# rayanirban/DiffSplitting

Hardware: AMD Instinct MI355X
Metric: sampled images/sec (2000-step 128x128 SR3) (higher is better)
Workload: dtype bf16; 1 GPU; sr_sr3_16_128: GaussianDiffusion.p_sample_loop, 16->128 SR3 UNet (97.8M params), T=2000 linear schedule; one step = UNet forward + posterior update of the batch; batch_per_gpu=16, global_batch=16, image=128x128x3, sample_steps=2000, parallelism=1 independent replicas, final RCCL all-gather, hipgraph=True, streams=1, noise=device Philox4x32-10, weights=random-init, seed 0

## Files before the change

### diffsplitting_amd/csrc/dsx_conv.hip

```cpp
#include "dsx_kernels.h"
#include <algorithm>
#include <cstdlib>
#include <mutex>
#include <type_traits>
#include <utility>

#ifndef DSX_WS_DEPTH_EXPR
#define DSX_WS_DEPTH_EXPR (bm == 64 ? 5 : (bm == 256 ? 2 : (ks == 1 ? 3 : 4)))
#endif
#ifndef DSX_PRE_RESID_EXPR
#define DSX_PRE_RESID_EXPR (NB == 1 && MB <= 2)
#endif
#ifndef DSX_PFF_EXPR
#define DSX_PFF_EXPR (NB == 2 ? 3 : 6)
#endif
#ifndef DSX_WS_K0_EXPR
#define DSX_WS_K0_EXPR 64
#endif
#ifndef DSX_EPI_PRIO_COND
#define DSX_EPI_PRIO_COND false
#endif
#ifndef DSX_STAMP_CVT_COND
#define DSX_STAMP_CVT_COND (tiC == 2 && gC == 0)
#endif
// ... 1075 lines not shown
  auto tile_pixel0 = [&](const TilePos& t) __attribute__((always_inline)) -> int {
    return (t.b * a.Ho + (t.ty << a.th_log2)) * a.Wo + (t.tx << a.tw_log2);
  };
  TilePos cur;
  {
    const int q1 = (int)fastdiv((unsigned)p0, a.mg_tiles_x);
    cur.b = (int)fastdiv((unsigned)p0, a.mg_per_img);
    cur.tx = p0 - q1 * a.tiles_x;
    cur.ty = q1 - cur.b * a.tiles_y;
  }
  TilePos nxt = cur;
  tile_advance(nxt);
  TilePos nn = nxt;
  tile_advance(nn);

  auto load_aff = [&](int b, int slot) __attribute__((always_inline)) {
    if (a.gn_scale == nullptr || tid * 4 >= C) return;
    float* dst = aff_base + (size_t)slot * (AFFB / 4);
    *(float4*)(dst + tid * 4) = *(const float4*)(a.gn_scale + (size_t)b * C + tid * 4);
    *(float4*)(dst + C + tid * 4) = *(const float4*)(a.gn_shift + (size_t)b * C + tid * 4);
  };
  TilePos n3 = nn;
  tile_advance(n3);
  load_aff(cur.b, 0);
  if (ntile > 1) load_aff(nxt.b, 1);
  if (ntile > 2) load_aff(nn.b, 2);

  constexpr int NR = 8 / CPU;
  const float4 zero4 = make_float4(0.f, 0.f, 0.f, 0.f);
  float4 addv[NB][2], affv[2];
  constexpr bool PRE_RESID = DSX_PRE_RESID_EXPR;
  uint4 residv[PRE_RESID ? MB : 1][NB][2][NR];
#pragma unroll
  for (int nb = 0; nb < NB; ++nb)
#pragma unroll
    for (int j = 0; j < 2; ++j) addv[nb][j] = zero4;
  if (a.bias && !a.film) {
#pragma unroll
    for (int nb = 0; nb < NB; ++nb)
#pragma unroll
      for (int j = 0; j < 2; ++j) addv[nb][j] = *(const float4*)(a.bias + nbase + 32 * nb + 4 * j);
  }
#pragma unroll
  for (int mb = 0; mb < (PRE_RESID ? MB : 1); ++mb)
#pragma unroll
    for (int nb = 0; nb < NB; ++nb)
#pragma unroll
      for (int ph = 0; ph < 2; ++ph)
#pragma unroll
        for (int q = 0; q < NR; ++q) residv[mb][nb][ph][q] = make_uint4(0u, 0u, 0u, 0u);
  affv[0] = affv[1] = zero4;
  auto prefetch_epilogue = [&](const TilePos& t, bool want_aff, int b_aff) __attribute__((always_inline)) {
    if (a.film) {
#pragma unroll
      for (int nb = 0; nb < NB; ++nb)
#pragma unroll
        for (int j = 0; j < 2; ++j)
          addv[nb][j] = *(const float4*)(a.film + (size_t)t.b * a.film_bs + nbase + 32 * nb + 4 * j);
    }
    if (PRE_RESID && a.resid) {
      const int r0 = tile_pixel0(t) * a.resid_ld;
#pragma unroll
      for (int mb = 0; mb < (PRE_RESID ? MB : 1); ++mb)
#pragma unroll
        for (int ph = 0; ph < 2; ++ph) {
          const DT* rp = (const DT*)a.resid + (r0 + rrow[mb] + ph * r16);
#pragma unroll
          for (int nb = 0; nb < NB; ++nb)
#pragma unroll
            for (int q = 0; q < NR; ++q) residv[mb][nb][ph][q] = *(const uint4*)(rp + 32 * nb + CPU * q);
        }
    }
    if (want_aff && a.gn_scale != nullptr && tid * 4 < C) {
      affv[0] = *(const float4*)(a.gn_scale + (size_t)b_aff * C + tid * 4);
      affv[1] = *(const float4*)(a.gn_shift + (size_t)b_aff * C + tid * 4);
    }
  };
  prefetch_epilogue(cur, ntile > 3, n3.b);

  constexpr bool PF_OK = !(NB == 2 && KS == 3);
  unsigned fin_pf_acc = 0u;
  if constexpr (PF_OK) fin_pf_acc = l2_prefetch_fold(l2_prefetch(a.pf, blockIdx.x, gridDim.x, tid, 256));
  if constexpr (KS == 1) {
    if (a.fin_on) {
      fin_pf_acc |= l2_prefetch_fold(l2_prefetch(a.fin.pf, blockIdx.x, gridDim.x, tid, 256));
      const int nitems = a.fin.B * a.fin.groups;
      for (int item = (int)blockIdx.x * 4 + wave; item < nitems; item += (int)gridDim.x * 4)
        gn_finalize_item<1>(a.fin, item % a.fin.B, item / a.fin.B, lane, nullptr);
    }
  }

  if constexpr (NBUF >= 3) {
    if (tid < 8) ((unsigned*)(lds + NBUF * BUFB + 3 * AFFB + NSLOT * RAWB))[tid] = 0u;
  }
  ws_barrier();
  if constexpr (NBUF == 2) ws_barrier();
  DSX_STAMP_T(0, tid == 0);
  int g = 0, ti = 0, aslot = 0;
  int ibuf = 0;
  constexpr int NPAIR = NSTEP / 2;
  constexpr int NF = 2 * MB;
  constexpr int FT = NPAIR * NF;
  constexpr int PFF = (DSX_PFF_EXPR) < FT ? (DSX_PFF_EXPR) : FT - 1;
  static_assert(PFF >= 1 && PFF < FT && PFF <= 15, "lgkmcnt is 4 bits");
  constexpr int RP = D > NSTEP ? D / NSTEP : 1;
  if constexpr (RP == 1) {
    for (int v = 0; v < total; ++v) {
      constexpr int R0 = 0;
#define DSX_WS_ITEM_NEXT continue
#include "dsx_conv_ws_item.inc"
#undef DSX_WS_ITEM_NEXT
    }
  } else {
    for (int v0 = 0; v0 < total; v0 += RP)
      static_for<RP>([&](auto rc_) __attribute__((always_inline)) {
        constexpr int R0 = decltype(rc_)::value * NSTEP;
        const int v = v0 + decltype(rc_)::value;
        if (v >= total) return;
#define DSX_WS_ITEM_NEXT return
#include "dsx_conv_ws_item.inc"
#undef DSX_WS_ITEM_NEXT
      });
  }
  if constexpr (PF_OK) l2_prefetch_retire(a.pf, fin_pf_acc);
}


template <typename DT, int KS, int NPH>
__global__ __launch_bounds__(512, 1) void k_conv_img(const ConvArgs a) {
  constexpr int KC = Chunk<DT>::KC;
  constexpr int CPU = Unit<DT>::N;
  constexpr int ES = (int)sizeof(DT);
  constexpr int TAPS = KS * KS, PAD = KS / 2, PW = 8 + 2 * PAD;
  constexpr int PIXB = 80;
  constexpr int RB = KS == 3 ? 896 : 640;
  constexpr int IMGB = PW * RB;
  constexpr int NSTEP = TAPS * 2;
  constexpr int D = NSTEP;
  constexpr int MAXP = NPH;
  constexpr bool ALLW = NPH == 2;
  static_assert(NSTEP % D == 0, "ring depth divides the steps of a phase");
  extern __shared__ __attribute__((aligned(16))) unsigned char lds[];

  const int tid = threadIdx.x, lane = tid & 63;
  const int wave = __builtin_amdgcn_readfirstlane(tid >> 6);
  const int li = lane & 31, lh = lane >> 5;
  const int nb = blockIdx.x % a.nblocks, b = blockIdx.x / a.nblocks;
  const int C = a.C0 + a.C1;
  const int nphase = NPH != 8 ? NPH : C / (8 * KC);
  unsigned char* img = lds + wave * (2 * IMGB);
  float* aff = (float*)(lds + 8 * 2 * IMGB) + wave * (8 * 2 * KC);

  DSX_STAMP(0);
  if (KS == 3) {
    for (int q = lane; q < 360; q += 64) {
      const int bufi = q >= 180, r = q - 180 * bufi, bp = r / 5, u = r - 5 * bp;
      int py, px2;
      if (bp < 10) { py = 0; px2 = bp; }
      else if (bp < 20) { py = 9; px2 = bp - 10; }
      else { py = 1 + ((bp - 20) >> 1); px2 = ((bp - 20) & 1) ? 9 : 0; }
      *(uint4*)(img + bufi * IMGB + py * RB + px2 * PIXB + u * 16) = make_uint4(0u, 0u, 0u, 0u);
    }
  }

  auto load_raw = [&](int p, uint4 (&raw)[4]) __attribute__((always_inline)) {
    const int c0 = (p * 8 + wave) * KC;
    const bool first = c0 < a.C0;
    const char* src = (const char*)(first ? a.src0 : a.src1);
    const int Cs = first ? a.C0 : a.C1, cl = first ? c0 : c0 - a.C0;
#pragma unroll
    for (int i = 0; i < 4; ++i) {
      const int q = lane + 64 * i, px = q >> 2, u = q & 3;
      raw[i] = *(const uint4*)(src + (((size_t)b * 64 + px) * Cs + cl + u * CPU) * ES);
    }
  };
  auto convert_store = [&](int p, const uint4 (&raw)[4]) __attribute__((always_inline)) {
    unsigned char* buf = img + (p & 1) * IMGB;
    const int u = lane & 3;
    float sc[CPU], sh[CPU];
    if (a.has_gn) {
#pragma unroll
      for (int j = 0; j < CPU; ++j) { sc[j] = aff[p * 2 * KC + u * CPU + j]; sh[j] = aff[p * 2 * KC + KC + u * CPU + j]; }
    }
#pragma unroll
    for (int i = 0; i < 4; ++i) {
      const int px = (lane + 64 * i) >> 2;
      float v[CPU];
      Unit<DT>::unpack(raw[i], v);
      if (a.has_gn) affine_vec(v, sc, sh);
      if (a.swish) swish_vec(v);
      *(uint4*)(buf + ((px >> 3) + PAD) * RB + ((px & 7) + PAD) * PIXB + u * 16) = Unit<DT>::pack(v);
    }
  };

  uint2 glo[MAXP], ghi[MAXP];
  float gg[MAXP], gb[MAXP];
  if (a.has_gn) {
#pragma unroll
    for (int p = 0; p < MAXP; ++p) {
      const int pp = p < nphase ? p : nphase - 1;
      const int c0 = (pp * 8 + wave) * KC, cb = c0 & ~63, c = cb + lane;
      const bool first = cb < a.C0;
      const char* part = (const char*)(first ? a.gn_part0 : a.gn_part1);
      const int nch = first ? a.gn_nchunk0 : a.gn_nchunk1, pf32 = first ? a.gn_pf32_0 : a.gn_pf32_1;
      const int Cs = first ? a.C0 : a.C1, cl = first ? c : c - a.C0;
      const char* e = part + (((size_t)b * nch) * Cs + cl) * (pf32 ? 8 : 16);
      glo[p] = *(const uint2*)e;
      ghi[p] = *(const uint2*)(e + 8);
      gg[p] = a.gn_gamma[c]; gb[p] = a.gn_beta[c];
    }
  }
  uint4 raw0[4], raw1[4];
  load_raw(0, raw0);
  if (nphase > 1) load_raw(1, raw1);

  const unsigned char* wbase = (const unsigned char*)a.wpack + (size_t)nb * a.kchunks * (NSTEP * 1024) + lane * 16;
  int pn = 0, sn = 0;
  auto load_w = [&]() __attribute__((always_inline)) -> uint4 {
    const uint4 v = *(const uint4*)(wbase + ((size_t)(pn * 8 + wave) * NSTEP + sn) * 1024);
    if (++sn == NSTEP) { sn = 0; ++pn; }
    return v;
  };
  uint4 wq[D], wq1[ALLW ? D : 1];
#pragma unroll
  for (int j = 0; j < D; ++j) wq[j] = load_w();
  if constexpr (ALLW) {
    if (nphase > 1) {
#pragma unroll
      for (int j = 0; j < D; ++j) wq1[j] = load_w();
    }
  }
  DSX_STAMP(1);

  if (a.has_gn) {
    const int cpg = C / a.gn_groups;
    double gs[MAXP], gq[MAXP];
#pragma unroll
    for (int p = 0; p < MAXP; ++p) {
      const int pp = p < nphase ? p : nphase - 1;
      const int cb = ((pp * 8 + wave) * KC) & ~63, c = cb + lane;
      const bool first = cb < a.C0;
      const int nch = first ? a.gn_nchunk0 : a.gn_nchunk1, pf32 = first ? a.gn_pf32_0 : a.gn_pf32_1;
      const double d0 = __builtin_bit_cast(double, ((unsigned long long)glo[p].y << 32) | glo[p].x);
      const double d1 = __builtin_bit_cast(double, ((unsigned long long)ghi[p].y << 32) | ghi[p].x);
      gs[p] = pf32 ? (double)__builtin_bit_cast(float, glo[p].x) : d0;
      gq[p] = pf32 ? (double)__builtin_bit_cast(float, glo[p].y) : d1;
      if (nch > 1 && p < nphase) {
        const char* part = (const char*)(first ? a.gn_part0 : a.gn_part1);
        const int Cs = first ? a.C0 : a.C1, cl = first ? c : c - a.C0;
        for (int k = 1; k < nch; ++k) {
          const size_t idx = (((size_t)b * nch + k) * Cs + cl) * 2;
          if (pf32) { const float2 v = *(const float2*)((const float*)part + idx); gs[p] += v.x; gq[p] += v.y; }
          else { const double2 v = *(const double2*)((const double*)part + idx); gs[p] += v.x; gq[p] += v.y; }
        }
      }
      const StatPivot& piv = first ? a.gn_piv0 : a.gn_piv1;
      if (piv.bias || piv.film)
        stat_unshift(gs[p], gq[p], (double)stat_pivot(piv, b, first ? c : c - a.C0), (double)(a.Hs * a.Ws));
    }
    const float inv_n = 1.0f / (64.0f * (float)cpg);
#pragma unroll
    for (int p = 0; p < MAXP; ++p) {
      if (p < nphase) {
        const int c0 = (p * 8 + wave) * KC, c = (c0 & ~63) + lane;
        float s = (float)gs[p], q = (float)gq[p];
        for (int o = 1; o < cpg; o <<= 1) { s += __shfl_xor(s, o, 64); q += __shfl_xor(q, o, 64); }
        const double mean = (double)s * (double)inv_n;
        double var = (double)q * (double)inv_n - mean * mean;
        if (var < 0) var = 0;
        const float rstd = __builtin_amdgcn_rsqf((float)var + a.gn_eps);
        const float meanf = (float)mean;
        if (c >= c0 && c < c0 + KC) {
          const float sc = rstd * gg[p];
          aff[p * 2 * KC + (c - c0)] = sc;
          aff[p * 2 * KC + KC + (c - c0)] = gb[p] - meanf * sc;
        }
      }
    }
  }
  const PfAcc pf_acc = l2_prefetch(a.pf, blockIdx.x, gridDim.x, tid, 512);
  DSX_STAMP(2);
  __builtin_amdgcn_s_waitcnt(0xC07F);
  convert_store(0, raw0);
  if (nphase > 1) convert_store(1, raw1);
  DSX_STAMP(3);

  int abase[2][KS];
#pragma unroll
  for (int mb = 0; mb < 2; ++mb) {
    const int m = mb * 32 + li;
#pragma unroll
    for (int dy = 0; dy < KS; ++dy) abase[mb][dy] = ((m >> 3) + dy) * RB + (m & 7) * PIXB + lh * 16;
  }
  f32x16 acc[2];
#pragma unroll
  for (int mb = 0; mb < 2; ++mb)
#pragma unroll
    for (int r = 0; r < 16; ++r) acc[mb][r] = 0.f;

  for (int p = 0; p < nphase; ++p) {
    const unsigned char* buf = img + (p & 1) * IMGB;
    if (p + 2 < nphase) load_raw(p + 2, raw0);
    const bool more = p + 1 < nphase;
    static_for<NSTEP>([&](auto sc_) __attribute__((always_inline)) {
      constexpr int s = decltype(sc_)::value;
      constexpr int tap = s >> 1, fs = s & 1, dy = tap / KS, dx = tap % KS;
      uint4 wcur = wq[s % D];
      if constexpr (ALLW) {
        if (p == 1) wcur = wq1[s % D];
      } else {
        if (more) wq[s % D] = load_w();
      }
#pragma unroll
      for (int mb = 0; mb < 2; ++mb) {
        const f32x4_t px = *(const f32x4_t*)(buf + abase[mb][dy] + dx * PIXB + fs * 32);
        acc[mb] = mfma_step<DT>(wcur, px, acc[mb]);
      }
    });
    if (p + 2 < nphase) convert_store(p + 2, raw0);
    DSX_STAMP(4 + p);
  }

  const int px = tid >> 3, cg = (tid & 7) * 4;
  const int n0 = nb * 32 + cg;
  const size_t opix = (size_t)b * 64 + px;
  float4 eb = make_float4(0.f, 0.f, 0.f, 0.f), ef = eb;
  float er[4] = {0.f, 0.f, 0.f, 0.f};
  if (a.bias) eb = *(const float4*)(a.bias + n0);
  if (a.film) ef = *(const float4*)(a.film + (size_t)b * a.film_bs + n0);
  if (a.resid) {
#pragma unroll
    for (int j = 0; j < 4; ++j) er[j] = act_load<DT>(a.resid, opix * a.resid_ld + n0 + j);
  }
  __syncthreads();
  DSX_STAMP(12);
  float* part = (float*)lds;
#pragma unroll
  for (int mb = 0; mb < 2; ++mb)
#pragma unroll
    for (int j = 0; j < 4; ++j)
      *(float4*)(part + ((wave * 2 + mb) * 64 + lane) * 20 + 4 * j) =
          make_float4(acc[mb][4 * j], acc[mb][4 * j + 1], acc[mb][4 * j + 2], acc[mb][4 * j + 3]);
  __syncthreads();
  DSX_STAMP(13);
  const int mbo = px >> 5, lo = (px & 31) + 32 * (cg >> 4), r0 = cg & 15;
  float x[4] = {0.f, 0.f, 0.f, 0.f};
#pragma unroll
  for (int w = 0; w < 8; ++w) {
    const float4 t = *(const float4*)(part + ((w * 2 + mbo) * 64 + lo) * 20 + r0);
    x[0] += t.x; x[1] += t.y; x[2] += t.z; x[3] += t.w;
  }
  x[0] += eb.x; x[1] += eb.y; x[2] += eb.z; x[3] += eb.w;
  x[0] += ef.x; x[1] += ef.y; x[2] += ef.z; x[3] += ef.w;
#pragma unroll
  for (int j = 0; j < 4; ++j) x[j] += er[j];
  const int okind = a.out_bf16;
  if (okind == 0) {
    *(float4*)((float*)a.out + opix * a.out_ld + n0) = make_float4(x[0], x[1], x[2], x[3]);
  } else {
    uint2 w2;
    if (okind == 1) { w2.x = pack_bf16x2(x[0], x[1]); w2.y = pack_bf16x2(x[2], x[3]); }
    else { w2.x = pack_f16x2(x[0], x[1]); w2.y = pack_f16x2(x[2], x[3]); }
    *(uint2*)((unsigned short*)a.out + opix * a.out_ld + n0) = w2;
  }
  DSX_STAMP(14);
  if (a.stat_part != nullptr) {
    float s1[4], s2[4];
#pragma unroll
    for (int j = 0; j < 4; ++j) { s1[j] = x[j]; s2[j] = x[j] * x[j]; }
#pragma unroll
    for (int o = 8; o < 64; o <<= 1)
#pragma unroll
      for (int j = 0; j < 4; ++j) { s1[j] += __shfl_xor(s1[j], o, 64); s2[j] += __shfl_xor(s2[j], o, 64); }
    __syncthreads();
    float* red = (float*)lds;
    if (lane < 8) {
#pragma unroll
      for (int j = 0; j < 4; ++j) { red[(wave * 32 + cg + j) * 2] = s1[j]; red[(wave * 32 + cg + j) * 2 + 1] = s2[j]; }
    }
    __syncthreads();
    if (tid < 64) {
      const int ch = tid >> 1, k = tid & 1;
      float t = 0.f;
#pragma unroll
      for (int w = 0; w < 8; ++w) t += red[(w * 32 + ch) * 2 + k];
      a.stat_part[((size_t)b * a.Cout + nb * 32 + ch) * 2 + k] = t;
    }
  }
  l2_prefetch_retire(a.pf, pf_acc);
  DSX_STAMP(15);
}

static size_t conv_img_lds(int dtype, int ks) {
  const int KC = dtype != 0 ? 32 : 16;
  const int pw = ks == 3 ? 10 : 8, rb = ks == 3 ? 896 : 640;
  return (size_t)8 * 2 * pw * rb + (size_t)8 * 8 * 2 * KC * sizeof(float);
}
bool conv_img_applicable(int dtype, int ks, int stride, const ConvArgs& a, bool gn, int gn_groups) {
  if (stride != 1 || a.up || !(ks == 1 || ks == 3)) return false;
  if (a.Hs != 8 || a.Ws != 8 || a.Ho != 8 || a.Wo != 8) return false;
  const int KC = dtype != 0 ? 32 : 16, C = a.C0 + a.C1;
  if (a.C0 % (8 * KC) || a.C1 % (8 * KC) || C / (8 * KC) > 8 || C < 8 * KC) return false;
  if (a.Cout % 32 || (a.out_ld & 3) || (a.resid && (a.resid_ld & 3))) return false;
  if (gn) {
    if (gn_groups < 1 || C % gn_groups) return false;
    const int cpg = C / gn_groups;
    if (cpg > 64 || (cpg & (cpg - 1)) || a.C0 % cpg) return false;
  }
  return true;
}


template <typename DT>
__global__ __launch_bounds__(256) void k_conv_first(const ConvArgs a) {
  constexpr bool F32 = sizeof(DT) == 4;
  constexpr int ES = (int)sizeof(DT);
  constexpr int KSTEP = F32 ? 2 : 16;
  constexpr int NS16 = 4;
  __shared__ __attribute__((aligned(16))) unsigned char sm[18 * 18 * 7 * 4 + 64 * 4];
  DT* patch = (DT*)sm;
  int* kofft = (int*)(sm + 18 * 18 * 7 * 4);

  const int tid = threadIdx.x, lane = tid & 63;
  const int wave = __builtin_amdgcn_readfirstlane(tid >> 6);
  const int li = lane & 31, lh = lane >> 5;
  const int Cin = a.C0 + a.C1, K = 9 * Cin;
  const int tiles_x = a.Wo >> 4, tiles_y = a.Ho >> 4;
  const int t = blockIdx.x % (tiles_x * tiles_y), b = blockIdx.x / (tiles_x * tiles_y);
  const int ty = t / tiles_x, tx = t - ty * tiles_x;
  const int oy0 = ty * 16, ox0 = tx * 16;
  const int NBLK = (a.Cout + 31) >> 5;

  for (int e = tid; e < 18 * 18 * Cin; e += 256) {
    const int c = e % Cin, pp = e / Cin, px = pp % 18, py = pp / 18;
    const int iy = oy0 + py - 1, ix = ox0 + px - 1;
    DT v = (DT)0.f;
    if (iy >= 0 && iy < a.Hs && ix >= 0 && ix < a.Ws) {
      const size_t pix = ((size_t)b * a.Hs + iy) * a.Ws + ix;
      v = c < a.C0 ? ((const DT*)a.src0)[pix * a.C0 + c] : ((const DT*)a.src1)[pix * a.C1 + (c - a.C0)];
    }
    patch[e] = v;
  }
  if (F32 && tid < 64) {
    const int k = tid < K ? tid : 0;
    const int tap = k / Cin, c = k - tap * Cin;
    kofft[tid] = ((tap / 3) * 18 + (tap % 3)) * Cin + c;
  }
  int koff[F32 ? 1 : NS16 * 8];
  if constexpr (!F32) {
#pragma unroll
    for (int s = 0; s < NS16; ++s)
#pragma unroll
      for (int j = 0; j < 8; ++j) {
        int k = 16 * s + 8 * lh + j;
        if (k >= K) k = 0;
        const int tap = k / Cin, c = k - tap * Cin;
        koff[s * 8 + j] = (((tap / 3) * 18 + (tap % 3)) * Cin + c) * 2;
      }
  }
  uint4 wf[F32 ? 1 : 2 * NS16];
  if constexpr (!F32) {
#pragma unroll
    for (int nb = 0; nb < 2; ++nb)
#pragma unroll
      for (int s = 0; s < NS16; ++s)
        wf[nb * NS16 + s] = nb < NBLK ? ((const uint4*)a.wpack)[(nb * NS16 + s) * 64 + lane] : make_uint4(0u, 0u, 0u, 0u);
  }
  __syncthreads();

  f32x16 acc[2][2];
#pragma unroll
  for (int mb = 0; mb < 2; ++mb)
#pragma unroll
    for (int nb = 0; nb < 2; ++nb)
#pragma unroll
      for (int r = 0; r < 16; ++r) acc[mb][nb][r] = 0.f;

#pragma unroll
  for (int mb = 0; mb < 2; ++mb) {
    const int m = (wave * 2 + mb) * 32 + li;
    const int base = ((m >> 4) * 18 + (m & 15)) * Cin;
    if constexpr (F32) {
      const int nsteps = (K + 1) >> 1;
      const float* wp = (const float*)a.wpack;
      for (int s = 0; s < nsteps; ++s) {
        const float pv = ((const float*)patch)[base + kofft[2 * s + lh]];
#pragma unroll
        for (int nb = 0; nb < 2; ++nb) {
          if (nb < NBLK) acc[mb][nb] = __builtin_amdgcn_mfma_f32_32x32x2f32(wp[(nb * 32 + s) * 64 + lane], pv, acc[mb][nb], 0, 0, 0);
        }
      }
    } else {
      const unsigned char* pb = (const unsigned char*)patch + base * 2;
#pragma unroll
      for (int s = 0; s < NS16; ++s) {
        unsigned w4[4];
#pragma unroll
        for (int q = 0; q < 4; ++q) {
          const unsigned lo = *(const unsigned short*)(pb + koff[s * 8 + 2 * q]);
          const unsigned hi = *(const unsigned short*)(pb + koff[s * 8 + 2 * q + 1]);
          w4[q] = lo | (hi << 16);
        }
        const f32x4_t px = __builtin_bit_cast(f32x4_t, make_uint4(w4[0], w4[1], w4[2], w4[3]));
#pragma unroll
        for (int nb = 0; nb < 2; ++nb)
          if (nb < NBLK) acc[mb][nb] = mfma_step<DT>(wf[nb * NS16 + s], px, acc[mb][nb]);
      }
    }
  }
  (void)KSTEP; (void)ES;

  const int okind = a.out_bf16;
#pragma unroll
  for (int nb = 0; nb < 2; ++nb) {
    const int nbase = nb * 32 + 16 * lh;
    if (nb >= NBLK) continue;
    float s1[16], s2[16];
#pragma unroll
    for (int r = 0; r < 16; ++r) { s1[r] = 0.f; s2[r] = 0.f; }
    const bool live = nbase < a.Cout;
#pragma unroll
    for (int mb = 0; mb < 2; ++mb) {
      const int m = (wave * 2 + mb) * 32 + li;
      const size_t opix = ((size_t)b * a.Ho + (oy0 + (m >> 4))) * a.Wo + (ox0 + (m & 15));
      float x[16], pv[16];
#pragma unroll
      for (int r = 0; r < 16; ++r) { x[r] = acc[mb][nb][r]; pv[r] = 0.f; }
      if (live) {
        if (a.bias) {
#pragma unroll
          for (int j = 0; j < 4; ++j) { const float4 tt = *(const float4*)(a.bias + nbase + 4 * j); pv[4 * j] = tt.x; pv[4 * j + 1] = tt.y; pv[4 * j + 2] = tt.z; pv[4 * j + 3] = tt.w; }
#pragma unroll
          for (int r = 0; r < 16; ++r) x[r] += pv[r];
        }
        store16<true>(a.out, opix * a.out_ld + nbase, x, okind, 16);
#pragma unroll
        for (int r = 0; r < 16; ++r) { const float d = x[r] - pv[r]; s1[r] += d; s2[r] += d * d; }
      }
    }
    if (a.stat_part != nullptr) {
      float w1 = row16_fold(s1, lane), w2 = row16_fold(s2, lane);
      w1 += __shfl_xor(w1, 16, 64);
      w2 += __shfl_xor(w2, 16, 64);
      const int nch = tiles_x * tiles_y * 4, chunk = t * 4 + wave;
      const int n = nbase + row16_fold_reg(li);
      if (li < 16 && n < a.Cout) {
        float* pp = a.stat_part + (((size_t)b * nch + chunk) * a.Cout + n) * 2;
        pp[0] = w1; pp[1] = w2;
      }
    }
  }
}

bool conv_first_applicable(int ks, int stride, const ConvArgs& a, bool gn) {
  const int C = a.C0 + a.C1;
  return ks == 3 && stride == 1 && !a.up && !gn && !a.swish && C >= 1 && C <= 7 && a.Cout >= 16 && a.Cout <= 64 &&
         (a.Cout & 15) == 0 && (a.Ho & 15) == 0 && (a.Wo & 15) == 0 && a.Ho == a.Hs && a.Wo == a.Ws && a.out_ld == a.Cout;
}
hipError_t launch_conv_first(int dtype, const ConvArgs& a, hipStream_t st) {
  const unsigned grid = (unsigned)(a.B * (a.Ho >> 4) * (a.Wo >> 4));
  if (dtype == 1) hipLaunchKernelGGL(k_conv_first<__bf16>, dim3(grid), dim3(256), 0, st, a);
  else if (dtype == 2) hipLaunchKernelGGL(k_conv_first<_Float16>, dim3(grid), dim3(256), 0, st, a);
  else hipLaunchKernelGGL(k_conv_first<float>, dim3(grid), dim3(256), 0, st, a);
  return hipGetLastError();
}

enum ConvFamily { FAM_MFMA, FAM_WS, FAM_IMG };
struct ConvVariant {
  int family, dtype, tile, ks, stride, cpg;
  void (*kern)(const ConvArgs);
  int block, lds_cap;
  int MB, WM, WN, NB;
  int max_px;
  int nit;
  int depth, nbuf;
  bool fuses_stats;
};
static constexpr int kLdsDefault = 64 * 1024, kLdsMax = 160 * 1024;
static constexpr int conv_cpg(int ks) { return ks == 1 ? 2 : 1; }
int conv_chunk_multiple(int ks) { return conv_cpg(ks); }

static constexpr int mfma_max_px(int bm, int ks, int stride, int cpg) {
  if (ks == 1) return bm;
  if (stride == 2) return 400;
  if (cpg == 2) return bm == 256 ? 324 : 220;
  return bm == 256 ? 400 : (bm == 128 ? 220 : 144);
}
template <typename DT, int TILE, int MB, int WM, int WN, int KS, int S = 1, int CPG = conv_cpg(KS)>
constexpr ConvVariant mfma_row() {
  constexpr bool G2 = KS == 3 && CPG == 2;
  constexpr int D = KS == 1 ? 4 : (G2 ? 6 : DSX_RING_DEPTH);
  constexpr int PX = mfma_max_px(32 * MB * WM, KS, S, CPG);
  constexpr int MI = (PX * 4 * CPG + 255) / 256;
  return {FAM_MFMA, Kind<DT>::value, TILE, KS, S, CPG, k_conv_mfma<DT, MB, WM, WN, KS, S, CPG, D, MI>, 256,
          G2 ? kLdsMax : kLdsDefault, MB, WM, WN, 1, PX, MI, 0, 2, MB <= 2};
}

static constexpr int kWsLoaderWaves = 4;
static constexpr int ws_max_px(int bm, int ks) { return ks == 1 ? bm : (bm == 256 ? 324 : (bm == 128 ? 180 : 108)); }
static constexpr int ws_depth(int bm, int ks, int cpg) {
#ifndef DSX_WS_DEPTH_C2_64
#define DSX_WS_DEPTH_C2_64 3
#endif
  if (ks == 3 && cpg == 2) return bm == 64 ? DSX_WS_DEPTH_C2_64 : 2;
  if (ks == 3 && cpg == 4) return 1;
  if (ks == 1 && cpg == 4) return bm == 64 ? 2 : 1;
  return DSX_WS_DEPTH_EXPR;
}
template <typename DT, int TILE, int MB, int WM, int WN, int NB, int KS, int CPG = conv_cpg(KS)>
constexpr ConvVariant ws_row() {
  constexpr int BM = 32 * MB * WM;
  constexpr int D = KS == 1 ? ((NB == 2 || MB == 4) ? DSX_RING_1X1_NB2 : DSX_RING_1X1_NB1) : ((NB == 2 || MB == 4) ? 6 : 18);
  constexpr int PX = ws_max_px(BM, KS);
  constexpr int NIT = (PX * 4 * CPG + kWsLoaderWaves * 64 - 1) / (kWsLoaderWaves * 64);
  constexpr int P = ws_depth(BM, KS, CPG);
  return {FAM_WS, Kind<DT>::value, TILE, KS, 1, CPG, k_conv_ws<DT, MB, WM, WN, NB, KS, CPG, D, NIT, P, kWsLoaderWaves>,
          256 + 64 * kWsLoaderWaves, kLdsMax, MB, WM, WN, NB, PX, NIT, P, ws_nbuf(BM, KS, NB, CPG), true};
}

template <typename DT, int KS, int NPH> constexpr ConvVariant img_row() {
  return {FAM_IMG, Kind<DT>::value, -1, KS, 1, NPH, k_conv_img<DT, KS, NPH>, 512, kLdsMax, 0, 0, 0, 0, 0, 0, 0, 0, true};
}

template <int N> struct ConvVariants {
  ConvVariant row[N];
  constexpr const ConvVariant* begin() const { return row; }
  constexpr const ConvVariant* end() const { return row + N; }
};
template <int... N> constexpr ConvVariants<(N + ...)> concat(const ConvVariants<N>&... parts) {
  ConvVariants<(N + ...)> out{};
  int n = 0;
  auto append = [&](const auto& p) { for (const ConvVariant& v : p) out.row[n++] = v; };
  (append(parts), ...);
  return out;
}

template <typename DT> constexpr ConvVariants<34> variants_of() {
  return {{
      mfma_row<DT, TILE_256x128, 8, 1, 4, 1>(), mfma_row<DT, TILE_256x128, 8, 1, 4, 3>(),
      mfma_row<DT, TILE_128x128, 4, 1, 4, 1>(), mfma_row<DT, TILE_128x128, 4, 1, 4, 3>(),
      mfma_row<DT, TILE_64x128, 2, 1, 4, 1>(), mfma_row<DT, TILE_64x128, 2, 1, 4, 3>(),
      mfma_row<DT, TILE_256x64, 4, 2, 2, 1>(), mfma_row<DT, TILE_256x64, 4, 2, 2, 3>(),
      mfma_row<DT, TILE_128x64, 2, 2, 2, 1>(), mfma_row<DT, TILE_128x64, 2, 2, 2, 3>(),
      mfma_row<DT, TILE_128x64, 2, 2, 2, 3, 1, 2>(),
      mfma_row<DT, TILE_64x64, 1, 2, 2, 1>(), mfma_row<DT, TILE_64x64, 1, 2, 2, 3>(),
      mfma_row<DT, TILE_64x64, 1, 2, 2, 3, 2>(),
      mfma_row<DT, TILE_128x32, 1, 4, 1, 1>(), mfma_row<DT, TILE_128x32, 1, 4, 1, 3>(),
      mfma_row<DT, TILE_128x32, 1, 4, 1, 3, 1, 2>(), mfma_row<DT, TILE_256x32, 2, 4, 1, 3, 1, 2>(),
      ws_row<DT, TILE_64x128, 2, 1, 4, 1, 1>(), ws_row<DT, TILE_64x128, 2, 1, 4, 1, 3>(),
      ws_row<DT, TILE_64x128, 2, 1, 4, 1, 1, 4>(),
      ws_row<DT, TILE_64x128, 2, 1, 4, 1, 3, 2>(),
      ws_row<DT, TILE_64x128, 2, 1, 4, 1, 3, 4>(),
      ws_row<DT, TILE_128x64, 2, 2, 2, 1, 1>(), ws_row<DT, TILE_128x64, 2, 2, 2, 1, 3>(),
      ws_row<DT, TILE_256x64, 4, 2, 2, 1, 3>(),
      ws_row<DT, TILE_64x64, 1, 2, 2, 1, 1>(), ws_row<DT, TILE_64x64, 1, 2, 2, 1, 3>(),
      img_row<DT, 1, 2>(), img_row<DT, 1, 4>(), img_row<DT, 1, 8>(),
      img_row<DT, 3, 2>(), img_row<DT, 3, 4>(), img_row<DT, 3, 8>(),
  }};
}
template <typename DT> constexpr ConvVariants<4> ws_nb2_variants() {
  return {{ws_row<DT, TILE_128x128, 2, 2, 2, 2, 1>(), ws_row<DT, TILE_128x128, 2, 2, 2, 2, 3>(),
           ws_row<DT, TILE_128x128, 2, 2, 2, 2, 1, 4>(), ws_row<DT, TILE_128x128, 2, 2, 2, 2, 3, 2>()}};
}
static constexpr auto kVariants = concat(variants_of<float>(), variants_of<__bf16>(), variants_of<_Float16>(),
                                         ws_nb2_variants<__bf16>(), ws_nb2_variants<_Float16>());

static constexpr int kKeySlots = 3 * 3 * (TILE_COUNT + 1) * 2 * 2 * 4;
static constexpr int key_slot(int family, int dtype, int tile, int ks, int stride, int cpg) {
  const int c = cpg == 1 ? 0 : (cpg == 2 ? 1 : (cpg == 4 ? 2 : (cpg == 8 ? 3 : -1)));
  if (family < 0 || family > FAM_IMG || dtype < 0 || dtype > 2 || tile < -1 || tile >= TILE_COUNT || (ks != 1 && ks != 3) ||
      (stride != 1 && stride != 2) || c < 0)
    return -1;
  return ((((family * 3 + dtype) * (TILE_COUNT + 1) + tile + 1) * 2 + ks / 2) * 2 + stride - 1) * 4 + c;
}
struct VariantIndex { short row[kKeySlots]; bool unique; };
static constexpr VariantIndex index_variants() {
  VariantIndex ix{};
  for (short& r : ix.row) r = -1;
  ix.unique = true;
  short n = 0;
  for (const ConvVariant& v : kVariants) {
    const int s = key_slot(v.family, v.dtype, v.tile, v.ks, v.stride, v.cpg);
    if (s < 0 || ix.row[s] >= 0) ix.unique = false;
    else ix.row[s] = n;
    ++n;
  }
  return ix;
}
static constexpr VariantIndex kIndex = index_variants();
static_assert(kIndex.unique, "kVariants: two rows share a key, or a key is outside key_slot's ranges");
static const ConvVariant* find_variant(int family, int dtype, int tile, int ks, int stride, int cpg) {
  const int s = key_slot(family, dtype, tile, ks, stride, cpg);
  return s >= 0 && kIndex.row[s] >= 0 ? &kVariants.row[kIndex.row[s]] : nullptr;
}

static constexpr bool variants_consistent() {
  for (const ConvVariant& a : kVariants) {
    const bool big = a.family != FAM_MFMA || (a.ks == 3 && a.cpg == 2);
    if (a.lds_cap != (big ? kLdsMax : kLdsDefault) || a.block != (a.family == FAM_MFMA ? 256 : 512)) return false;
    for (const ConvVariant& b : kVariants) {
      if (a.tile == b.tile && (a.MB * a.WM != b.MB * b.WM || a.WN * a.NB != b.WN * b.NB)) return false;
      if (a.tile == b.tile && a.family == b.family && (a.WM != b.WM || a.fuses_stats != b.fuses_stats)) return false;
    }
  }
  return true;
}
static_assert(variants_consistent(), "kVariants: wrong LDS limit / block size, or two layouts for one tile");

ConvTileInfo conv_tile_info(int tile, bool ws) {
  for (const ConvVariant& v : kVariants)
    if (v.family == (ws ? FAM_WS : FAM_MFMA) && v.tile == tile) return {32 * v.MB * v.WM, 32 * v.WN * v.NB, v.WM, v.fuses_stats};
  return {0, 0, 0, false};
}
// ... 168 lines not shown
```

Measured before the change: 2.929 images/s.

## Make first conv persistent with double-buffered patch prefetch and padded LDS layout

The first 3x3 conv kernel becomes persistent: each workgroup loops over several 16x16 tiles, with the grid capped. While the current tile's MFMA work runs, it prefetches the next tile's input patch into registers and writes it into a second LDS buffer. The LDS patch uses a per-pixel dword pitch and padded row pitch to cut bank conflicts, and bias is staged in LDS. This is meant to hide global load latency and cut per-workgroup setup. The cost is more registers and LDS and fewer workgroups on a kernel that is a small share of the UNet step.

```diff
diff --git a/diffsplitting_amd/csrc/dsx_conv.hip b/diffsplitting_amd/csrc/dsx_conv.hip
--- a/diffsplitting_amd/csrc/dsx_conv.hip
+++ b/diffsplitting_amd/csrc/dsx_conv.hip
@@ -1510,52 +1510,48 @@
 }
 
 
+#ifndef DSX_FIRST_TPW
+#define DSX_FIRST_TPW 4
+#endif
+static constexpr int kFirstMaxWgs = 512;
+__host__ __device__ constexpr int first_pix_dw(int cin, int es) { return ((cin * es + 3) >> 2) | 1; }
+__host__ __device__ constexpr int first_row_dw(int pdw) { return ((18 * pdw - 16 + 31) & ~31) + 16; }
+static_assert(first_row_dw(1) == 48 && first_row_dw(3) == 80 && first_row_dw(5) == 112 && first_row_dw(7) == 144, "row pitch");
+static constexpr int kFirstBufBytes = 18 * first_row_dw(7) * 4;
+
 template <typename DT>
-__global__ __launch_bounds__(256) void k_conv_first(const ConvArgs a) {
+__global__ __launch_bounds__(256, 2) void k_conv_first(const ConvArgs a) {
   constexpr bool F32 = sizeof(DT) == 4;
   constexpr int ES = (int)sizeof(DT);
-  constexpr int KSTEP = F32 ? 2 : 16;
   constexpr int NS16 = 4;
-  __shared__ __attribute__((aligned(16))) unsigned char sm[18 * 18 * 7 * 4 + 64 * 4];
-  DT* patch = (DT*)sm;
-  int* kofft = (int*)(sm + 18 * 18 * 7 * 4);
+  __shared__ __attribute__((aligned(16))) unsigned char sm[2 * kFirstBufBytes + 64 * 4 + 64 * 4];
+  int* kofft = (int*)(sm + 2 * kFirstBufBytes);
+  float* biasl = (float*)(sm + 2 * kFirstBufBytes + 64 * 4);
 
   const int tid = threadIdx.x, lane = tid & 63;
   const int wave = __builtin_amdgcn_readfirstlane(tid >> 6);
   const int li = lane & 31, lh = lane >> 5;
-  const int Cin = a.C0 + a.C1, K = 9 * Cin;
-  const int tiles_x = a.Wo >> 4, tiles_y = a.Ho >> 4;
-  const int t = blockIdx.x % (tiles_x * tiles_y), b = blockIdx.x / (tiles_x * tiles_y);
-  const int ty = t / tiles_x, tx = t - ty * tiles_x;
-  const int oy0 = ty * 16, ox0 = tx * 16;
+  const int C0 = a.C0, C1 = a.C1, Cin = C0 + C1, K = 9 * Cin;
+  const int Pdw = first_pix_dw(Cin, ES), Rdw = first_row_dw(Pdw);
+  const int tiles_x = a.Wo >> 4, tiles_y = a.Ho >> 4, tpi = tiles_x * tiles_y;
+  const int total = a.B * tpi, step = (int)gridDim.x;
   const int NBLK = (a.Cout + 31) >> 5;
 
-  for (int e = tid; e < 18 * 18 * Cin; e += 256) {
-    const int c = e % Cin, pp = e / Cin, px = pp % 18, py = pp / 18;
-    const int iy = oy0 + py - 1, ix = ox0 + px - 1;
-    DT v = (DT)0.f;
-    if (iy >= 0 && iy < a.Hs && ix >= 0 && ix < a.Ws) {
-      const size_t pix = ((size_t)b * a.Hs + iy) * a.Ws + ix;
-      v = c < a.C0 ? ((const DT*)a.src0)[pix * a.C0 + c] : ((const DT*)a.src1)[pix * a.C1 + (c - a.C0)];
-    }
-    patch[e] = v;
-  }
-  if (F32 && tid < 64) {
+  if (tid < 64) {
     const int k = tid < K ? tid : 0;
     const int tap = k / Cin, c = k - tap * Cin;
-    kofft[tid] = ((tap / 3) * 18 + (tap % 3)) * Cin + c;
-  }
-  int koff[F32 ? 1 : NS16 * 8];
-  if constexpr (!F32) {
-#pragma unroll
-    for (int s = 0; s < NS16; ++s)
-#pragma unroll
-      for (int j = 0; j < 8; ++j) {
-        int k = 16 * s + 8 * lh + j;
-        if (k >= K) k = 0;
-        const int tap = k / Cin, c = k - tap * Cin;
-        koff[s * 8 + j] = (((tap / 3) * 18 + (tap % 3)) * Cin + c) * 2;
-      }
+    kofft[tid] = ((tap / 3) * Rdw + (tap % 3) * Pdw) * 4 + c * ES;
+    biasl[tid] = (a.bias != nullptr && tid < a.Cout) ? a.bias[tid] : 0.f;
+  }
+  int ppy[2], ppx[2];
+  unsigned padr[2];
+  bool pown[2];
+#pragma unroll
+  for (int j = 0; j < 2; ++j) {
+    const int p = tid + 256 * j;
+    pown[j] = p < 18 * 18;
+    ppy[j] = p / 18; ppx[j] = p - 18 * ppy[j];
+    padr[j] = (unsigned)((ppy[j] * Rdw + ppx[j] * Pdw) * 4);
   }
   uint4 wf[F32 ? 1 : 2 * NS16];
   if constexpr (!F32) {
@@ -1565,89 +1561,147 @@
       for (int s = 0; s < NS16; ++s)
         wf[nb * NS16 + s] = nb < NBLK ? ((const uint4*)a.wpack)[(nb * NS16 + s) * 64 + lane] : make_uint4(0u, 0u, 0u, 0u);
   }
+
+  DT pv_[2][7];
+  bool pin[2];
+  const void* const src_any = C0 > 0 ? a.src0 : a.src1;
+  auto load_patch = [&](int tile) {
+    const int b = tile / tpi, t = tile - b * tpi;
+    const int ty = t / tiles_x, tx = t - ty * tiles_x;
+#pragma unroll
+    for (int j = 0; j < 2; ++j) {
+      const int iy = ty * 16 + ppy[j] - 1, ix = tx * 16 + ppx[j] - 1;
+      pin[j] = pown[j] && iy >= 0 && iy < a.Hs && ix >= 0 && ix < a.Ws;
+      const size_t pix = pin[j] ? ((size_t)b * a.Hs + iy) * a.Ws + ix : 0;
+#pragma unroll
+      for (int c = 0; c < 7; ++c) {
+        const DT* base = (const DT*)(c < C0 ? a.src0 : a.src1);
+        size_t idx = c < C0 ? pix * C0 + c : pix * C1 + (c - C0);
+        if (c >= Cin) { base = (const DT*)src_any; idx = 0; }
+        pv_[j][c] = base[idx];
+      }
+    }
+  };
+  auto write_patch = [&](unsigned char* buf) {
+#pragma unroll
+    for (int j = 0; j < 2; ++j)
+      if (pown[j]) {
+#pragma unroll
+        for (int c = 0; c < 7; ++c)
+          if (c < Cin) *(DT*)(buf + padr[j] + c * ES) = pin[j] ? pv_[j][c] : (DT)0.f;
+      }
+  };
+
+  int tile = blockIdx.x;
+  load_patch(tile);
   __syncthreads();
-
-  f32x16 acc[2][2];
-#pragma unroll
-  for (int mb = 0; mb < 2; ++mb)
-#pragma unroll
-    for (int nb = 0; nb < 2; ++nb)
-#pragma unroll
-      for (int r = 0; r < 16; ++r) acc[mb][nb][r] = 0.f;
-
-#pragma unroll
-  for (int mb = 0; mb < 2; ++mb) {
-    const int m = (wave * 2 + mb) * 32 + li;
-    const int base = ((m >> 4) * 18 + (m & 15)) * Cin;
-    if constexpr (F32) {
-      const int nsteps = (K + 1) >> 1;
-      const float* wp = (const float*)a.wpack;
-      for (int s = 0; s < nsteps; ++s) {
-        const float pv = ((const float*)patch)[base + kofft[2 * s + lh]];
-#pragma unroll
-        for (int nb = 0; nb < 2; ++nb) {
-          if (nb < NBLK) acc[mb][nb] = __builtin_amdgcn_mfma_f32_32x32x2f32(wp[(nb * 32 + s) * 64 + lane], pv, acc[mb][nb], 0, 0, 0);
-        }
-      }
-    } else {
-      const unsigned char* pb = (const unsigned char*)patch + base * 2;
-#pragma unroll
-      for (int s = 0; s < NS16; ++s) {
-        unsigned w4[4];
-#pragma unroll
-        for (int q = 0; q < 4; ++q) {
-          const unsigned lo = *(const unsigned short*)(pb + koff[s * 8 + 2 * q]);
-          const unsigned hi = *(const unsigned short*)(pb + koff[s * 8 + 2 * q + 1]);
-          w4[q] = lo | (hi << 16);
-        }
-        const f32x4_t px = __builtin_bit_cast(f32x4_t, make_uint4(w4[0], w4[1], w4[2], w4[3]));
-#pragma unroll
-        for (int nb = 0; nb < 2; ++nb)
-          if (nb < NBLK) acc[mb][nb] = mfma_step<DT>(wf[nb * NS16 + s], px, acc[mb][nb]);
-      }
-    }
-  }
-  (void)KSTEP; (void)ES;
-
-  const int okind = a.out_bf16;
-#pragma unroll
-  for (int nb = 0; nb < 2; ++nb) {
-    const int nbase = nb * 32 + 16 * lh;
-    if (nb >= NBLK) continue;
-    float s1[16], s2[16];
-#pragma unroll
-    for (int r = 0; r < 16; ++r) { s1[r] = 0.f; s2[r] = 0.f; }
-    const bool live = nbase < a.Cout;
+  unsigned koff[F32 ? 1 : NS16 * 4];
+  if constexpr (!F32) {
+#pragma unroll
+    for (int s = 0; s < NS16; ++s)
+#pragma unroll
+      for (int q = 0; q < 4; ++q)
+        koff[s * 4 + q] = (unsigned)kofft[16 * s + 8 * lh + 2 * q] | ((unsigned)kofft[16 * s + 8 * lh + 2 * q + 1] << 16);
+  }
+  write_patch(sm);
+  int cur = 0;
+
+  for (;;) {
+    __syncthreads();
+    const unsigned char* patch = sm + cur * kFirstBufBytes;
+    const int next = tile + step;
+    const bool has_next = next < total;
+    if (has_next) load_patch(next);
+
+    const int b = tile / tpi, t = tile - b * tpi;
+    const int ty = t / tiles_x, tx = t - ty * tiles_x;
+    const int oy0 = ty * 16, ox0 = tx * 16;
+
+    f32x16 acc[2][2];
+#pragma unroll
+    for (int mb = 0; mb < 2; ++mb)
+#pragma unroll
+      for (int nb = 0; nb < 2; ++nb)
+#pragma unroll
+        for (int r = 0; r < 16; ++r) acc[mb][nb][r] = 0.f;
+
 #pragma unroll
     for (int mb = 0; mb < 2; ++mb) {
       const int m = (wave * 2 + mb) * 32 + li;
-      const size_t opix = ((size_t)b * a.Ho + (oy0 + (m >> 4))) * a.Wo + (ox0 + (m & 15));
-      float x[16], pv[16];
-#pragma unroll
-      for (int r = 0; r < 16; ++r) { x[r] = acc[mb][nb][r]; pv[r] = 0.f; }
-      if (live) {
-        if (a.bias) {
-#pragma unroll
-          for (int j = 0; j < 4; ++j) { const float4 tt = *(const float4*)(a.bias + nbase + 4 * j); pv[4 * j] = tt.x; pv[4 * j + 1] = tt.y; pv[4 * j + 2] = tt.z; pv[4 * j + 3] = tt.w; }
-#pragma unroll
-          for (int r = 0; r < 16; ++r) x[r] += pv[r];
-        }
-        store16<true>(a.out, opix * a.out_ld + nbase, x, okind, 16);
-#pragma unroll
-        for (int r = 0; r < 16; ++r) { const float d = x[r] - pv[r]; s1[r] += d; s2[r] += d * d; }
-      }
-    }
-    if (a.stat_part != nullptr) {
-      float w1 = row16_fold(s1, lane), w2 = row16_fold(s2, lane);
-      w1 += __shfl_xor(w1, 16, 64);
-      w2 += __shfl_xor(w2, 16, 64);
-      const int nch = tiles_x * tiles_y * 4, chunk = t * 4 + wave;
-      const int n = nbase + row16_fold_reg(li);
-      if (li < 16 && n < a.Cout) {
-        float* pp = a.stat_part + (((size_t)b * nch + chunk) * a.Cout + n) * 2;
-        pp[0] = w1; pp[1] = w2;
-      }
-    }
+      const unsigned char* pb = patch + ((m >> 4) * Rdw + (m & 15) * Pdw) * 4;
+      if constexpr (F32) {
+        const int nsteps = (K + 1) >> 1;
+        const float* wp = (const float*)a.wpack;
+        for (int s = 0; s < nsteps; ++s) {
+          const float pv = *(const float*)(pb + kofft[2 * s + lh]);
+#pragma unroll
+          for (int nb = 0; nb < 2; ++nb) {
+            if (nb < NBLK) acc[mb][nb] = __builtin_amdgcn_mfma_f32_32x32x2f32(wp[(nb * 32 + s) * 64 + lane], pv, acc[mb][nb], 0, 0, 0);
+          }
+        }
+      } else {
+#pragma unroll
+        for (int s = 0; s < NS16; ++s) {
+          unsigned w4[4];
+#pragma unroll
+          for (int q = 0; q < 4; ++q) {
+            const unsigned lo = *(const unsigned short*)(pb + (koff[s * 4 + q] & 0xffffu));
+            const unsigned hi = *(const unsigned short*)(pb + (koff[s * 4 + q] >> 16));
+            w4[q] = lo | (hi << 16);
+          }
+          const f32x4_t px = __builtin_bit_cast(f32x4_t, make_uint4(w4[0], w4[1], w4[2], w4[3]));
+#pragma unroll
+          for (int nb = 0; nb < 2; ++nb)
+            if (nb < NBLK) acc[mb][nb] = mfma_step<DT>(wf[nb * NS16 + s], px, acc[mb][nb]);
+        }
+      }
+    }
+
+    if (has_next) write_patch(sm + (cur ^ 1) * kFirstBufBytes);
+
+    const int okind = a.out_bf16;
+#pragma unroll
+    for (int nb = 0; nb < 2; ++nb) {
+      const int nbase = nb * 32 + 16 * lh;
+      if (nb >= NBLK) continue;
+      float s1[16], s2[16], pv[16];
+#pragma unroll
+      for (int r = 0; r < 16; ++r) { s1[r] = 0.f; s2[r] = 0.f; }
+#pragma unroll
+      for (int j = 0; j < 4; ++j) { const float4 tt = *(const float4*)(biasl + nbase + 4 * j); pv[4 * j] = tt.x; pv[4 * j + 1] = tt.y; pv[4 * j + 2] = tt.z; pv[4 * j + 3] = tt.w; }
+      const bool live = nbase < a.Cout;
+#pragma unroll
+      for (int mb = 0; mb < 2; ++mb) {
+        const int m = (wave * 2 + mb) * 32 + li;
+        const size_t opix = ((size_t)b * a.Ho + (oy0 + (m >> 4))) * a.Wo + (ox0 + (m & 15));
+        float x[16];
+#pragma unroll
+        for (int r = 0; r < 16; ++r) x[r] = acc[mb][nb][r];
+        if (live) {
+          if (a.bias) {
+#pragma unroll
+            for (int r = 0; r < 16; ++r) x[r] += pv[r];
+          }
+          store16<true>(a.out, opix * a.out_ld + nbase, x, okind, 16);
+#pragma unroll
+          for (int r = 0; r < 16; ++r) { const float d = x[r] - pv[r]; s1[r] += d; s2[r] += d * d; }
+        }
+      }
+      if (a.stat_part != nullptr) {
+        float w1 = row16_fold(s1, lane), w2 = row16_fold(s2, lane);
+        w1 += __shfl_xor(w1, 16, 64);
+        w2 += __shfl_xor(w2, 16, 64);
+        const int nch = tpi * 4, chunk = t * 4 + wave;
+        const int n = nbase + row16_fold_reg(li);
+        if (li < 16 && n < a.Cout) {
+          float* pp = a.stat_part + (((size_t)b * nch + chunk) * a.Cout + n) * 2;
+          pp[0] = w1; pp[1] = w2;
+        }
+      }
+    }
+    if (!has_next) break;
+    tile = next;
+    cur ^= 1;
   }
 }
 
@@ -1657,7 +1711,8 @@
          (a.Cout & 15) == 0 && (a.Ho & 15) == 0 && (a.Wo & 15) == 0 && a.Ho == a.Hs && a.Wo == a.Ws && a.out_ld == a.Cout;
 }
 hipError_t launch_conv_first(int dtype, const ConvArgs& a, hipStream_t st) {
-  const unsigned grid = (unsigned)(a.B * (a.Ho >> 4) * (a.Wo >> 4));
+  const int total = a.B * (a.Ho >> 4) * (a.Wo >> 4);
+  const unsigned grid = (unsigned)std::min((total + DSX_FIRST_TPW - 1) / DSX_FIRST_TPW, kFirstMaxWgs);
   if (dtype == 1) hipLaunchKernelGGL(k_conv_first<__bf16>, dim3(grid), dim3(256), 0, st, a);
   else if (dtype == 2) hipLaunchKernelGGL(k_conv_first<_Float16>, dim3(grid), dim3(256), 0, st, a);
   else hipLaunchKernelGGL(k_conv_first<float>, dim3(grid), dim3(256), 0, st, a);
```

Result: no change. 2.913 images/s (-0.5%).

## Split weight prefetch around halo zeroing and drop epilogue barriers via per-wave LDS reuse

Applied to the files above, without the earlier changes.

Each wave's halo-zeroing loop is now a straight-line store pattern indexed by lane. The initial weight-register loads are split into halves and spread around the GroupNorm prologue and the convert_store phases, fenced by sched_barriers, so global loads overlap other work. In the epilogue each wave parks its partial sums in its own image buffers and the stat reduction uses the aff region, which removes two __syncthreads. Timing stamps are added, and correctness depends on the LDS sizing assertions and on wave-private buffers being safe to overwrite without a barrier.

```diff
diff --git a/diffsplitting_amd/csrc/dsx_conv.hip b/diffsplitting_amd/csrc/dsx_conv.hip
--- a/diffsplitting_amd/csrc/dsx_conv.hip
+++ b/diffsplitting_amd/csrc/dsx_conv.hip
@@ -1251,16 +1251,7 @@
   float* aff = (float*)(lds + 8 * 2 * IMGB) + wave * (8 * 2 * KC);
 
   DSX_STAMP(0);
-  if (KS == 3) {
-    for (int q = lane; q < 360; q += 64) {
-      const int bufi = q >= 180, r = q - 180 * bufi, bp = r / 5, u = r - 5 * bp;
-      int py, px2;
-      if (bp < 10) { py = 0; px2 = bp; }
-      else if (bp < 20) { py = 9; px2 = bp - 10; }
-      else { py = 1 + ((bp - 20) >> 1); px2 = ((bp - 20) & 1) ? 9 : 0; }
-      *(uint4*)(img + bufi * IMGB + py * RB + px2 * PIXB + u * 16) = make_uint4(0u, 0u, 0u, 0u);
-    }
-  }
+  DSX_STAMP_T(16 + wave, lane == 0);
 
   auto load_raw = [&](int p, uint4 (&raw)[4]) __attribute__((always_inline)) {
     const int c0 = (p * 8 + wave) * KC;
@@ -1320,15 +1311,22 @@
     if (++sn == NSTEP) { sn = 0; ++pn; }
     return v;
   };
+  constexpr int DH = D / 2;
   uint4 wq[D], wq1[ALLW ? D : 1];
 #pragma unroll
-  for (int j = 0; j < D; ++j) wq[j] = load_w();
-  if constexpr (ALLW) {
-    if (nphase > 1) {
-#pragma unroll
-      for (int j = 0; j < D; ++j) wq1[j] = load_w();
-    }
-  }
+  for (int j = 0; j < DH; ++j) wq[j] = load_w();
+  if (KS == 3) {
+    if (lane < 36) {
+      const int py = lane < 10 ? 0 : lane < 20 ? 9 : 1 + ((lane - 20) >> 1);
+      const int px2 = lane < 10 ? lane : lane < 20 ? lane - 10 : ((lane - 20) & 1) * 9;
+      unsigned char* z = img + py * RB + px2 * PIXB;
+#pragma unroll
+      for (int bufi = 0; bufi < 2; ++bufi)
+#pragma unroll
+        for (int u = 0; u < 5; ++u) *(uint4*)(z + bufi * IMGB + u * 16) = make_uint4(0u, 0u, 0u, 0u);
+    }
+  }
+  __builtin_amdgcn_sched_barrier(0);
   DSX_STAMP(1);
 
   if (a.has_gn) {
@@ -1377,11 +1375,27 @@
       }
     }
   }
+  __builtin_amdgcn_sched_barrier(0);
+#pragma unroll
+  for (int j = DH; j < D; ++j) wq[j] = load_w();
   const PfAcc pf_acc = l2_prefetch(a.pf, blockIdx.x, gridDim.x, tid, 512);
+  __builtin_amdgcn_sched_barrier(0);
   DSX_STAMP(2);
   __builtin_amdgcn_s_waitcnt(0xC07F);
   convert_store(0, raw0);
+  if constexpr (ALLW) {
+    __builtin_amdgcn_sched_barrier(0);
+#pragma unroll
+    for (int j = 0; j < DH; ++j) wq1[j] = load_w();
+    __builtin_amdgcn_sched_barrier(0);
+  }
   if (nphase > 1) convert_store(1, raw1);
+  if constexpr (ALLW) {
+    __builtin_amdgcn_sched_barrier(0);
+#pragma unroll
+    for (int j = DH; j < D; ++j) wq1[j] = load_w();
+    __builtin_amdgcn_sched_barrier(0);
+  }
   DSX_STAMP(3);
 
   int abase[2][KS];
@@ -1431,22 +1445,23 @@
 #pragma unroll
     for (int j = 0; j < 4; ++j) er[j] = act_load<DT>(a.resid, opix * a.resid_ld + n0 + j);
   }
-  __syncthreads();
+  static_assert(2 * IMGB >= 2 * 64 * 20 * (int)sizeof(float), "a wave's parked partial sums fit its own image buffers");
+  float* part = (float*)img;
+#pragma unroll
+  for (int mb = 0; mb < 2; ++mb)
+#pragma unroll
+    for (int j = 0; j < 4; ++j)
+      *(float4*)(part + (mb * 64 + lane) * 20 + 4 * j) =
+          make_float4(acc[mb][4 * j], acc[mb][4 * j + 1], acc[mb][4 * j + 2], acc[mb][4 * j + 3]);
   DSX_STAMP(12);
-  float* part = (float*)lds;
-#pragma unroll
-  for (int mb = 0; mb < 2; ++mb)
-#pragma unroll
-    for (int j = 0; j < 4; ++j)
-      *(float4*)(part + ((wave * 2 + mb) * 64 + lane) * 20 + 4 * j) =
-          make_float4(acc[mb][4 * j], acc[mb][4 * j + 1], acc[mb][4 * j + 2], acc[mb][4 * j + 3]);
+  DSX_STAMP_T(24 + wave, lane == 0);
   __syncthreads();
   DSX_STAMP(13);
   const int mbo = px >> 5, lo = (px & 31) + 32 * (cg >> 4), r0 = cg & 15;
   float x[4] = {0.f, 0.f, 0.f, 0.f};
 #pragma unroll
   for (int w = 0; w < 8; ++w) {
-    const float4 t = *(const float4*)(part + ((w * 2 + mbo) * 64 + lo) * 20 + r0);
+    const float4 t = *(const float4*)((const float*)(lds + w * (2 * IMGB)) + (mbo * 64 + lo) * 20 + r0);
     x[0] += t.x; x[1] += t.y; x[2] += t.z; x[3] += t.w;
   }
   x[0] += eb.x; x[1] += eb.y; x[2] += eb.z; x[3] += eb.w;
@@ -1471,8 +1486,8 @@
     for (int o = 8; o < 64; o <<= 1)
 #pragma unroll
       for (int j = 0; j < 4; ++j) { s1[j] += __shfl_xor(s1[j], o, 64); s2[j] += __shfl_xor(s2[j], o, 64); }
-    __syncthreads();
-    float* red = (float*)lds;
+    static_assert(8 * 8 * 2 * KC * sizeof(float) >= 8 * 32 * 2 * sizeof(float), "`red` fits the aff tables (conv_img_lds)");
+    float* red = (float*)(lds + 8 * 2 * IMGB);
     if (lane < 8) {
 #pragma unroll
       for (int j = 0; j < 4; ++j) { red[(wave * 32 + cg + j) * 2] = s1[j]; red[(wave * 32 + cg + j) * 2 + 1] = s2[j]; }
```

New measurement: 3.002 images/s before, 3.026 images/s after, median of 6. Within noise of the previous version (+0.8%).
